# veronicaguerrini/BFQzip

Hardware: AMD Instinct MI355X
Metric: Mbases/s end-to-end (eBWT+cluster+LF), reads and results resident in HBM (higher is better)
Workload: dtype u64

## Files before the change

bfqzip_amd/_lib.py:

```python
import ctypes as C
import os
import subprocess

_HERE = os.path.dirname(os.path.abspath(__file__))
LIB_PATH = os.path.join(_HERE, "libbfqhip.so")
_LIB = None

SYMBOLS = [
    "bfq_default_params", "bfq_create", "bfq_create_error", "bfq_destroy", "bfq_set_params",
    "bfq_last_error", "bfq_stream", "bfq_device_count", "bfq_pick_device", "bfq_device_lease", "bfq_device_release",
    "bfq_phase_enable", "bfq_phase", "bfq_phase_report", "bfq_output_prefault", "bfq_fastq_rows_estimate", "bfq_build_ebwt", "bfq_count_reads",
    "bfq_smooth_invert", "bfq_run_reads", "bfq_run_reads_device", "bfq_fetch_ebwt",
    "bfq_fastq_out_bound", "bfq_fastq_build_ebwt", "bfq_fastq_run", "bfq_fastq_run_streams",
    "bfq_smooth_invert_fastq", "bfq_fastq_run_job", "bfq_host_alloc", "bfq_host_free",
    "bfq_text_count_lines", "bfq_text_nth_newline", "bfq_file_put", "bfq_file_map", "bfq_file_unmap", "bfq_fastq_build_ebwt_fd", "bfq_smooth_invert_fastq_fd",
    "bfq_glob_begin", "bfq_glob_local_text", "bfq_glob_pile_counts", "bfq_glob_init_out", "bfq_glob_run_pile", "bfq_glob_finish",
    "bfq_synth_default", "bfq_synth_total", "bfq_synth_host", "bfq_synth_device", "bfq_synth_fastq",
    "bfq_posbin_geometry", "bfq_radix_geometry", "bfq_prof_enable", "bfq_prof_reset", "bfq_prof_count", "bfq_prof_get", "bfq_prof_trace_select", "bfq_prof_trace",
    "bfq_stream_bound", "bfq_stream_raw_len", "bfq_stream_compress", "bfq_stream_decompress",
    "bfq_stream_reserve", "bfq_stream_compress_device", "bfq_stream_ebwt_decode",
    "bfq_names_compress", "bfq_names_compress_device",
    "bfq_quals_compress", "bfq_quals_compress_device",
    "bfq_fastq_restore_bound", "bfq_fastq_restore", "bfq_fastq_restore_fd",
    "bfq_reorder_key", "bfq_fastq_reorder", "bfq_fastq_reorder_fd",
    "bfq_perm_bound", "bfq_perm_reads", "bfq_perm_encode", "bfq_perm_decode",
    "bfq_fastq_reorder_keep", "bfq_fastq_reorder_keep_fd", "bfq_fastq_unreorder", "bfq_fastq_unreorder_fd",
    "bfq_fastq_restore_ordered", "bfq_fastq_restore_ordered_fd",
    "bfq_fastq_restore_groups", "bfq_stream_members", "bfq_fastq_restore_grouped", "bfq_fastq_restore_grouped_fd",
    "bfq_fastq_compare", "bfq_fastq_compare_fd",
    "bfq_bgzf_probe", "bfq_bgzf_index", "bfq_bgzf_inflate", "bfq_bgzf_inflate_device", "bfq_bgzf_inflate_fd",
    "bfq_bgzf_deflate_bound", "bfq_bgzf_deflate_host", "bfq_bgzf_deflate", "bfq_bgzf_deflate_device", "bfq_bgzf_deflate_fd",
    "bfq_fastq_restore_bgzf_fd",
    "bfq_gzip_probe", "bfq_gzip_measure", "bfq_gzip_inflate", "bfq_gzip_inflate_device", "bfq_gzip_inflate_fd", "bfq_gzip_inflate_host",
# ... 247 lines not shown
        L.bfq_gzip_host_error.restype = C.c_char_p
        L.bfq_gzip_host_error.argtypes = []
        pbo, pbs, a3 = C.POINTER(BamOpts), C.POINTER(BamStats), C.POINTER(u64)
        L.bfq_bam_default_opts.restype = None
        L.bfq_bam_default_opts.argtypes = [pbo]
        L.bfq_bam_probe.argtypes = [vp, u64]
        L.bfq_bam_measure.argtypes = [vp, vp, u64, pbo, a3, a3, pbs]
        L.bfq_bam_to_fastq.argtypes = [vp, vp, u64, pbo, C.POINTER(vp), a3, a3, a3, pbs]
        L.bfq_bam_to_fastq_device.argtypes = [vp, vp, u64, pbo, C.POINTER(vp), a3, a3, a3, pbs]
        L.bfq_bam_to_fastq_fd.argtypes = [vp, C.c_int, u64, pbo, C.POINTER(C.c_int), a3, a3, pbs]
        L.bfq_bam_to_fastq_host.argtypes = [vp, u64, pbo, C.POINTER(vp), a3, a3, a3, pbs]
        L.bfq_bam_host_error.restype = C.c_char_p
        L.bfq_bam_host_error.argtypes = []
        L.bfq_fastq_restore_bgzf_fd.argtypes = [vp, C.c_int, u64, C.c_int, u64, C.c_int, u64, C.c_int, u64, C.c_int, C.c_int, pu64, pu64, pu64]
        L.bfq_posbin_geometry.argtypes = [u64, C.POINTER(u64), C.POINTER(C.c_int)]
        L.bfq_radix_geometry.argtypes = [u64, C.POINTER(u64), C.POINTER(u64)]
        L.bfq_prof_enable.argtypes = [vp, C.c_int]
        L.bfq_prof_reset.argtypes = [vp]
        L.bfq_prof_count.argtypes = [vp]
        L.bfq_prof_trace_select.argtypes = [vp, C.c_int]
        L.bfq_prof_trace.restype = C.c_int64
        L.bfq_prof_trace.argtypes = [vp, vp, u64]
        L.bfq_prof_get.argtypes = [vp, C.c_int, C.c_char_p, C.c_int, C.POINTER(C.c_double),
                                   C.POINTER(u64), C.POINTER(C.c_double)]
        _LIB = L
    return _LIB
```

bfqzip_amd/csrc/bfq_api.hip:

```cpp
#include <math.h>
#include <time.h>
#include <stdlib.h>
#include <stdio.h>
#include <string.h>
#include <unistd.h>
#include <errno.h>
#include <algorithm>
#include <new>
#include "bfq_internal.h"
#include "bfq_synth.h"
#include "bfq_device.h"
#include "bfq_rank.h"
#include "bfq_posbin.h"

const char *const BFQ_KERNEL_NAMES[K_NUM] = {
    "k_text_from_reads", "k_pack3", "k_build_keys", "k_radix_hist", "k_scan", "k_radix_scatter", "k_huge_round",
    "k_cluster_big", "k_refine_chunk", "k_refine_big", "k_emit_bwt", "k_lf_count", "k_lf_build", "k_lcp_flags",
    "k_cluster", "k_invert_count", "k_invert", "k_synth", "k_fastq", "k_bfs", "k_codec", "misc",
    "k_restore_index", "k_fq_format_lines", "k_reorder_keys", "k_reorder_gather",
    "k_fq_format_ordered", "k_perm_pack", "k_perm_invert", "k_posbin_l1", "k_posbin_l2", "k_posbin_apply",
    "k_cmp_check", "k_cmp_compare", "k_cmp_emit", "k_bgzf_inflate", "k_bgzf_deflate"};

static thread_local std::string g_createErr;

void bfq_ctx::reserveBegin(size_t bytes)
{
    bytes = (bytes + 0xFFFFF) & ~(size_t)0xFFFFF;
    if (wsThread || bytes <= ws.cap || (wsLimit() && bytes > wsLimit())) return;
    wsPendBytes = bytes; wsPend = nullptr;
    const int dev = device;
    wsThread = new std::thread([this, dev, bytes] {
        struct timespec t0, t1;
        clock_gettime(CLOCK_MONOTONIC, &t0);
        void *p = nullptr;
        if (hipSetDevice(dev) != hipSuccess || hipMalloc(&p, bytes) != hipSuccess) { (void)hipGetLastError(); p = nullptr; }
        clock_gettime(CLOCK_MONOTONIC, &t1);
// ... 229 lines not shown
extern "C" int64_t bfq_prof_trace(bfq_ctx *c, float *ms, uint64_t cap)
{
    if (!c) return BFQ_E_ARG;
    const size_t k = std::min<size_t>(cap, c->profTrace.size());
    if (ms && k) memcpy(ms, c->profTrace.data(), k * sizeof(float));
    return (int64_t)c->profTrace.size();
}
extern "C" int bfq_prof_count(bfq_ctx *c) { (void)c; return K_NUM; }
extern "C" int bfq_posbin_geometry(uint64_t n_rows, uint64_t *window, int *bin_shift)
{
    const int s = bfq_posbin_shift(n_rows);
    if (window) *window = BFQ_PB_W;
    if (bin_shift) *bin_shift = s;
    return s >= 0 ? BFQ_OK : BFQ_E_ARG;
}
extern "C" int bfq_radix_geometry(uint64_t n_rows, uint64_t *tile_rows, uint64_t *block_rows)
{
    if (tile_rows) *tile_rows = BFQ_RS_TILE;
    if (block_rows) *block_rows = bfq_radix_block_elems(n_rows);
    return BFQ_OK;
}
extern "C" int bfq_prof_get(bfq_ctx *c, int idx, char *name, int cap, double *ms, uint64_t *launches, double *bytes)
{
    if (!c || idx < 0 || idx >= K_NUM) return BFQ_E_ARG;
    if (name && cap > 0) { strncpy(name, BFQ_KERNEL_NAMES[idx], cap - 1); name[cap - 1] = 0; }
    if (ms) *ms = c->profMs[idx];
    if (launches) *launches = c->profLaunches[idx];
    if (bytes) *bytes = c->profBytes[idx];
    return BFQ_OK;
}

static void check_counters(bfq_ctx *c)
{
    const DevCounters &h = c->h_cnt;
    if (h.errSymbol) throw BfqError{BFQ_E_SYMBOL, "symbol outside {A,C,G,T,N,terminator}"};
    if (h.errTooLong) throw BfqError{BFQ_E_TOO_LONG, "read longer than BFQ_MAX_READ_LEN"};
    if (h.errInvert) throw BfqError{BFQ_E_NOT_EBWT, "LF walk did not close: not an eBWT of a read collection"};
    if (h.mismatch) throw BfqError{BFQ_E_NOT_EBWT, "eBWT is not in #_i<#_j<A<C<G<N<T suffix order"};
    if (h.errFreq3) throw BfqError{BFQ_E_FREQ3, "three frequent symbols in a cluster (bfq_int.cpp:505 assert); raise -f"};
}
static void finish_call(bfq_ctx *c, bfq_stats *st = nullptr)
{
    c->fetchCounters();
    c->profCollect();
    check_counters(c);
    if (!st) return;
    const u64 *s = c->h_cnt.stats;
    st->num_clust = s[0]; st->num_clust_discarded = s[1]; st->num_clust_amb_discarded = s[2];
    st->num_clust_mod = s[3]; st->num_clust_alleq = s[4]; st->bases_inside = s[5];
    st->qs_smoothed = s[6]; st->modified = s[7];
    st->n_rows = c->n; st->n_reads = c->N;
    st->n_segments = c->h_cnt.nSegs; st->n_big_segments = c->h_cnt.bigTotal + c->h_cnt.bigCount;
}

static size_t ws_need(u64 n, u64 N, u64 extra)
{
    const u64 nb = ceil_div(n + 1, bfq_radix_block_elems(n)) + 8;
    size_t need = 0;
    need += 4 * (n + 256) + 24 * (n / 256 + 2) + 4096;
    need += 8 * bfq_t3_alloc(n / 21 + 3);
// ... 210 lines not shown
    if (!n) return;
    u8 *dna = c->alloc<u8>(n + 64), *qs = c->alloc<u8>(n + 64);
    if (N) KLAUNCH(c, K_MISC, 4.0 * (double)(n - N), k_lines_init, bfq_grid(N, 16), 256, d_bases, d_quals, d_roff, N, c->P.B, dna, qs);
    u8 *in = c->alloc<u8>(n + 64);
    bfq_lcp_flags(c, c->d_lcp, n, c->P.K, in);
    ClusterPos pm{c->call.d_w12, c->call.d_text3, dna, qs, c->P.B};
    RankIndex none{nullptr, n};
    bfq_clusters(c, none, c->d_bwt, c->d_qual, in, n, &pm);
    if (N) KLAUNCH(c, K_MISC, 4.0 * (double)(n - N), k_lines_strip, bfq_grid(N, 16), 256, (const u8 *)dna, (const u8 *)qs, d_roff, N, d_out_bases, d_out_quals);
}

static size_t posbins_room_needed(u64 n)
{
    const size_t pb = bfq_posbins_need(n);
    if (pb == ~(size_t)0) return pb;
    return pb + 3 * (n + 64 + 256) + 24 * (n / 256 + 8) + (1u << 20);
}
static void steps34_posbins(bfq_ctx *c, const u64 *d_roff, u8 *d_out_bases, u8 *d_out_quals)
{
    const u64 n = c->n, N = c->N;
    if (!n) return;
    u8 *editQual = c->alloc<u8>(n + 64), *repl = c->alloc<u8>(n + 64);
    HIP_CHECK(hipMemcpyAsync(editQual, c->d_qual, n, hipMemcpyDeviceToDevice, c->stream));
    HIP_CHECK(hipMemsetAsync(repl, 0, n + 64, c->stream));
    {
        const size_t mk = c->mark();
        u8 *in = c->alloc<u8>(n + 64);
        bfq_lcp_flags(c, c->d_lcp, n, c->P.K, in);
        ClusterPos pm{c->call.d_w12, c->call.d_text3, nullptr, nullptr, c->P.B, editQual, repl};
        RankIndex none{nullptr, n};
        bfq_clusters(c, none, c->d_bwt, c->d_qual, in, n, &pm);
        c->release(mk);
    }
    bfq_posbins(c, const_cast<u64 *>(c->call.d_w12), repl, editQual, n, d_roff, N, c->P.B, d_out_bases, d_out_quals);
}

static void steps_capped(bfq_ctx *c, const u8 *d_bases, const u8 *d_quals, const u64 *d_roff, u64 N, u64 total, u8 *dna, u8 *qs)
{
    const u64 n = total + N;
    if (n >= (1ull << BFQ_POS_BITS)) throw BfqError{BFQ_E_ARG, "collection too large (2^37 rows)"};
    c->n = n; c->N = N;
    c->d_bwt = c->d_qual = nullptr; c->d_lcp = nullptr; c->d_gcnt = nullptr;
    if (!n) return;
    if (c->P.K < 1) throw BfqError{BFQ_E_NOMEM, "the capped mode needs -k >= 1 (with -k 0 every row is in one cluster): raise the workspace cap"};
// ... 1014 lines not shown
```

bfqzip_amd/csrc/bfq_host.cpp:

```cpp
#include <errno.h>
#include <fcntl.h>
#include <stdio.h>
#include <stdlib.h>
#include <string.h>
#include <sched.h>
#include <sys/file.h>
#include <sys/mman.h>
#include <sys/stat.h>
#include <time.h>
#include <unistd.h>
#include <algorithm>
#include <atomic>
#include <condition_variable>
#include <mutex>
#include <string>
#include <thread>
#include <vector>
#include "bfq_internal_host.h"
#include "bfq_reorder.h"
#include "bfq_perm.h"
#include "bfq_bgzf.h"

static double now_s()
{
// ... 13 lines not shown
            char *end = nullptr;
            double x = strtod(v, &end);
            if (end && (*end == 'G' || *end == 'g')) x *= 1073741824.0;
            else if (end && (*end == 'M' || *end == 'm')) x *= 1048576.0;
            else if (end && (*end == 'K' || *end == 'k')) x *= 1024.0;
            return (unsigned long long)x;
        };
        e.trace = getenv("BFQ_TRACE") != nullptr;
        e.piles = getenv("BFQ_PILES") ? (atoi(getenv("BFQ_PILES")) == 2 ? 2 : atoi(getenv("BFQ_PILES")) ? 1 : -1) : 0;
        e.pilesSplit = getenv("BFQ_PILES_SPLIT") != nullptr;
        e.noOverlap = getenv("BFQ_NO_OVERLAP") != nullptr;
        e.noLengthGuess = getenv("BFQ_NO_LENGTH_GUESS") != nullptr;
        e.posMode = geti("BFQ_POSMODE", 0) != 0;
        e.posBins = geti("BFQ_POSBINS", 1) != 0;
        e.fuseKeys = geti("BFQ_FUSEKEYS", 1) != 0;
        e.ioThreads = geti("BFQ_IO_THREADS", 0);
        e.prefaultThreads = geti("BFQ_PREFAULT_THREADS", -1);
        e.hugeCap = getu("BFQ_HUGE_CAP", 0);
        e.wsCap = getu("BFQ_WS_CAP", 0);
        e.device = getenv("BFQ_DEVICE") ? atoi(getenv("BFQ_DEVICE")) : -1;
        e.fakeDevices = geti("BFQ_FAKE_DEVICES", 0);
        e.lease = geti("BFQ_LEASE", 1) != 0;
        if (const char *d = getenv("BFQ_LEASE_DIR")) e.leaseDir = d;
        e.noOutmap = getenv("BFQ_NO_OUTMAP") != nullptr;
        e.compact = geti("BFQ_COMPACT", 0) != 0;
        e.prefaultPause = geti("BFQ_PREFAULT_PAUSE", 0) != 0;
        e.compactWin = getu("BFQ_COMPACT_WIN", 0);
        e.compactRing = getu("BFQ_COMPACT_RING", 0);
        e.bgzfBatch = getu("BFQ_BGZF_BATCH", 0);
        e.dnaStatic = geti("BFQ_DNA_STATIC", 0);
// ... 536 lines not shown
```

bfqzip_amd/csrc/bfq_internal.h:

```cpp
#pragma once
#include <stdlib.h>
#include <errno.h>
#include <unistd.h>
#include <hip/hip_runtime.h>
#include <stdint.h>
#include <functional>
#include <new>
#include <optional>
#include <string>
#include <vector>
#include <thread>
#include "../../include/bfqzip_hip.h"
#include "bfq_common.h"
#include "bfq_internal_host.h"
#include "bfq_arena.h"

#define HIP_CHECK(expr)                                                                        \
    do {                                                                                       \
        hipError_t e__ = (expr);                                                               \
        if (e__ != hipSuccess)                                                                 \
            throw BfqError{BFQ_E_HIP, std::string(#expr) + ": " + hipGetErrorString(e__)};     \
    } while (0)

enum BfqKernel {
    K_TEXT = 0, K_PACK, K_KEYS, K_RADIX_HIST, K_SCAN, K_RADIX_SCATTER, K_HUGE_ROUND, K_CLUSTER_BIG,
    K_REFINE_WAVE, K_REFINE_BIG, K_EMIT, K_RANK_BUILD, K_RANK_FINAL, K_LCP_FLAGS, K_CLUSTER,
    K_INVERT_COUNT, K_INVERT, K_SYNTH, K_FASTQ, K_BFS, K_CODEC, K_MISC, K_RESTORE, K_FQ_FORMAT, K_RO_KEYS, K_RO_GATHER,
    K_FQ_FORMAT_ORD, K_PERM_PACK, K_PERM_INVERT, K_POSBIN_L1, K_POSBIN_L2, K_POSBIN_APPLY,
    K_CMP_CHECK, K_CMP_COMPARE, K_CMP_EMIT, K_BGZF, K_DEFLATE, K_NUM
};
extern const char *const BFQ_KERNEL_NAMES[K_NUM];

struct ProfRec { int id; hipEvent_t a, b; double bytes; };

#define BFQ_IO_MAX_WORKERS 16
#define BFQ_IO_STAGE_BYTES (16u << 20)

struct DevCounters {
    u64 stats[8];
    u64 bigCount;
    u64 errSymbol;
    u64 errInvert;
    u64 errFreq3;
    u64 errTooLong;
    u64 tot[6];
    u64 mismatch;
    u64 nSegs;
    u64 errFastq;
    u64 hugeCount;
    u64 hugeRows;
    u64 bigClusters;
    u64 bigTotal;
    u64 pad[5];
};

struct RankIndex {
    u64 *lfq;
    u64 n;
};

struct CallState {
    bool piles = false;
    bool capped = false;
    u64 cappedPileRows = 0;
    bool keepRecs = false;
    const u64 *d_w12 = nullptr, *d_text3 = nullptr;
    size_t keepMark = 0;
    size_t writeHint = 0;
// ... 259 lines not shown
struct PileText { u8 *T8, *Q8; u64 *text3; };
void bfq_step1_piles(bfq_ctx *c, const u8 *d_bases, const u8 *d_quals, const u64 *d_roff, u64 N, u64 total, int termOut, bfq_stats *st,
                     const PileText *pre = nullptr, u64 capTarget = 0);
size_t bfq_ws_need_piles(u64 n, u64 N, u64 cap, u64 extra, bool lean = false);
struct PileRows { u64 m; u8 *bwt, *qs; u16 *lcp; const u64 *w12; };
u64 bfq_run_one_pile(bfq_ctx *c, const u8 *T8, const u8 *Q8, const u64 *text3, u64 n, u32 s, u32 s2, int termOut, PileRows *out);
void bfq_pile_pair_counts(bfq_ctx *c, const u8 *T8, u64 n, u64 *counts36);
void bfq_pack_text(bfq_ctx *c, const u8 *T8, u64 n, u64 *text3, u64 nwords);

RankIndex bfq_rank_build(bfq_ctx *c, const u8 *bwt, const u8 *qs, u64 n, int term, const u32 *gcnt = nullptr);
u64 *bfq_symbol_scans(bfq_ctx *c, const u8 *bwt, u64 n, int term, const u32 *gcntIn, u32 *gcntOut);
void bfq_rank_blocks(bfq_ctx *c, const u8 *bwt, u64 n, int term, const u64 *scanned, u64 *rank);
void bfq_lcp_flags(bfq_ctx *c, const u16 *lcp, u64 n, int K, u8 *in);
void bfq_lcp_from_bwt(bfq_ctx *c, const u8 *bwt, u64 n, u64 N, int term, u16 *lcp, u32 *gcntOut = nullptr,
                      const u64 *rankGiven = nullptr, u64 ringEntries = 0);
struct ClusterPos { const u64 *w12; const u64 *text3; u8 *outSym, *outQual; int B; u8 *editQual = nullptr, *repl = nullptr; };
struct ClusterRank { const u64 *rankBlk; u64 F[6]; u8 *qual, *repl; };
void bfq_clusters(bfq_ctx *c, const RankIndex &R, const u8 *bwt, const u8 *qual, const u8 *in, u64 n, const ClusterPos *pm = nullptr,
                  const ClusterRank *rm = nullptr);
#define BFQ_COMPACT_LCP_WIN (256ull << 20)
size_t bfq_ws_need_compact(bfq_ctx *c, u64 n, u64 N, u64 extra, bool haveLcp, size_t resident);
void bfq_steps234_compact(bfq_ctx *c, const u8 *bwt, u8 *qual, HostRef lcp, int lcp_bytes, u64 n, u64 N, u64 *d_roff, u32 *lens,
                          u8 **ob, u8 **oq, u64 extra, size_t resident);
void bfq_invert_count(bfq_ctx *c, const RankIndex &R, u64 N, u32 *lens);
void bfq_fixed_offsets(bfq_ctx *c, u64 N, u64 L, u64 *d_roff);
void bfq_invert(bfq_ctx *c, const RankIndex &R, u64 N, const u64 *d_roff, int B, u8 *out_bases, u8 *out_quals, u64 first = 0,
                u64 count = ~0ull, bool lines = false);
bool bfq_is_pinned(const void *p);
size_t bfq_posbins_need(u64 n);
void bfq_posbins(bfq_ctx *c, u64 *w12, const u8 *repl, const u8 *editQual, u64 n, const u64 *d_roff, u64 N, int B, u8 *outSym, u8 *outQual);

// ... 37 lines not shown
```

bfqzip_amd/csrc/bfq_internal_host.h:

```cpp
#pragma once
#include <stdint.h>
#include <atomic>
#include <string>
#include "../../include/bfqzip_hip.h"

struct BfqError {
    int code;
    std::string msg;
};

struct BfqEnv {
    bool trace = false;
    int piles = 0;
    bool pilesSplit = false;
    bool noOverlap = false;
    bool noLengthGuess = false;
    bool posMode = false;
    bool posBins = true;
    bool fuseKeys = true;
    int ioThreads = 0;
    int prefaultThreads = -1;
    unsigned long long hugeCap = 0;
    unsigned long long wsCap = 0;
    int device = -1;
    int fakeDevices = 0;
    bool lease = true;
    std::string leaseDir;
    bool compact = false;
    int dnaStatic = 0;
    int dnacK = 0, dnacH = 0, dnacW = 0, dnacSkip = -1;
    unsigned long long compactRing = 0;
    unsigned long long compactWin = 0;
    bool prefaultPause = false;
// ... 19 lines not shown
```

bfqzip_amd/csrc/k_cluster.hip:

```cpp
#include <stdlib.h>
#include "bfq_internal.h"
#include "bfq_device.h"
#include "bfq_rank.h"
#include "bfq_rankblk.h"

__global__ __launch_bounds__(256) void k_lcp_flags(const u16 *__restrict__ lcp, u64 n, int K, u8 *__restrict__ in)
{
    const u64 ngroups = (n + 7) / 8;
    for (u64 g = (u64)blockIdx.x * blockDim.x + threadIdx.x; g < ngroups; g += (u64)gridDim.x * blockDim.x) {
        u64 r0 = g * 8;
        int l[10];
        if (r0 >= 1 && r0 + 9 <= n) {
            u64 a = *(const u64 *)(lcp + r0 - 1), b = *(const u64 *)(lcp + r0 + 3);
            u32 c = *(const u32 *)(lcp + r0 + 7);
#pragma unroll
            for (int k = 0; k < 4; k++) { l[k] = (int)((a >> (16 * k)) & 0xFFFF); l[4 + k] = (int)((b >> (16 * k)) & 0xFFFF); }
            l[8] = (int)(c & 0xFFFF); l[9] = (int)(c >> 16);
        } else {
#pragma unroll
            for (int k = 0; k < 10; k++) { u64 r = r0 + k; l[k] = (r >= 1 && r - 1 < n) ? (int)lcp[r - 1] : 0; }
        }
        u64 out = 0;
#pragma unroll
        for (int k = 0; k < 8; k++) {
// ... 183 lines not shown
                else if (ch == symbPrec[1]) { set_mod(a, j, Freq[1]); st.modb++; }
            } else if (b == Freq[0] || b == Freq[1]) {
                set_qual(a, j, newqs); st.qs++;
            } else if (newqs < (int)(signed char)a.qual[j]) {
                set_qual(a, j, newqs); st.qs++;
            }
        }
    } else {
        st.amb++;
    }
    return false;
}

#define CL_CHUNK 4096
#define CL_WROWS (CL_CHUNK / 4)
__global__ __launch_bounds__(256) void k_cluster(ClusterArgs a, u64 nchunks)
{
    __shared__ u32 shst[8];
    __shared__ u16 starts[4][CL_WROWS];
    __shared__ u32 wn[4];
    const u32 lane = bfq_lane(), w = threadIdx.x >> 6;
    if (threadIdx.x < 8) shst[threadIdx.x] = 0;
    ClStat st = {0, 0, 0, 0, 0, 0, 0, 0};
    for (u64 ch = blockIdx.x; ch < nchunks; ch += gridDim.x) {
        const u64 r0 = ch * CL_CHUNK + (u64)w * CL_WROWS + (u64)lane * (CL_WROWS / 64);
        u32 bits = 0;
        if (r0 < a.n) {
            uint4 x = *(const uint4 *)(a.in + r0);
            u32 wds[4] = {x.x, x.y, x.z, x.w};
#pragma unroll
            for (int q = 0; q < 4; q++)
#pragma unroll
                for (int b = 0; b < 4; b++) bits |= ((wds[q] >> (8 * b)) & 1u) << (4 * q + b);
            if (r0 + 16 > a.n) bits &= (1u << (u32)(a.n - r0)) - 1u;
        }
        {
            const u32 zb = ~bits & 0xFFFFu;
            const u64 any = __ballot(zb != 0);
// ... 18 lines not shown
            u64 r = ch * CL_CHUNK + starts[ww][idx];
            if (process_cluster_body(a, r - 1, st)) a.bigStart[atomicAdd(&a.cnt->bigClusters, 1ull)] = r;
        }
        __syncthreads();
    }
    if (st.clust) atomicAdd(&shst[0], st.clust);
    if (st.disc) atomicAdd(&shst[1], st.disc);
    if (st.amb) atomicAdd(&shst[2], st.amb);
    if (st.mod) atomicAdd(&shst[3], st.mod);
    if (st.alleq) atomicAdd(&shst[4], st.alleq);
    if (st.bases) atomicAdd(&shst[5], st.bases);
    if (st.qs) atomicAdd(&shst[6], st.qs);
    if (st.modb) atomicAdd(&shst[7], st.modb);
    __syncthreads();
    if (threadIdx.x < 8 && shst[threadIdx.x]) atomicAdd(&a.cnt->stats[threadIdx.x], (u64)shst[threadIdx.x]);
}

struct BigState {
    u64 start, end;
    u64 freq[5];
    u32 low, sum, mx, fr0, fr1;
    int mode, newqs;
    u32 sym0, sym1;
};
#define CB_TILE 65536
#define CB_GRID 2048

#define CB_FOR_ROWS(...)                                                                               \
    for (u64 g0 = (ts & ~15ull) + (u64)threadIdx.x * 16; g0 <= te; g0 += 256 * 16) {                  \
        const uint4 xb4 = *(const uint4 *)(a.bwt + g0), xq4 = *(const uint4 *)(a.qual + g0);          \
// ... 209 lines not shown
    ClusterArgs a;
    a.R = R; a.bwt = bwt; a.qual = qual; a.in = in; a.n = n;
    a.rankBlk = rm ? rm->rankBlk : nullptr; a.editQual = rm ? rm->qual : pm ? pm->editQual : nullptr; a.repl = rm ? rm->repl : pm ? pm->repl : nullptr;
    for (int s = 0; s < 6; s++) a.F[s] = rm ? rm->F[s] : 0;
    a.w12 = pm ? pm->w12 : nullptr; a.text3 = pm ? pm->text3 : nullptr;
    a.outSym = pm ? pm->outSym : nullptr; a.outQual = pm ? pm->outQual : nullptr; a.B = pm ? pm->B : 0;
    a.m = c->P.m; a.v = c->P.v; a.f = c->P.f; a.t = c->P.t; a.term = c->P.term & 0xFF; a.M = c->P.M; a.ext = c->P.ext;
    a.powtab = c->d_powtab; a.qthr = c->d_qthr; a.qthrLo = c->qthrLo; a.qthrN = c->qthrN;
    a.cnt = c->d_cnt;
    size_t mk = c->mark();
    HIP_CHECK(hipMemsetAsync(&c->d_cnt->bigClusters, 0, sizeof(u64), c->stream));
    a.bigStart = c->alloc<u64>(n / CL_BIG + 2);
    a.big = c->alloc<BigState>(n / CL_BIG + 2);
    a.firstOut = c->alloc<u16>(n / CL_WROWS + 8);
    u64 nchunks = ceil_div(n, CL_CHUNK);
    KLAUNCH(c, K_CLUSTER, 4.125 * (double)n, k_cluster, bfq_grid(nchunks, 1), 256, a, nchunks);
    KLAUNCH(c, K_CLUSTER_BIG, 0.0, k_big_extent, 1024, 256, a);
    KLAUNCH(c, K_CLUSTER_BIG, 0.0, k_big_count, CB_GRID, 256, a);
    KLAUNCH(c, K_CLUSTER_BIG, 0.0, k_big_decide, 64, 256, a);
    KLAUNCH(c, K_CLUSTER_BIG, 0.0, k_big_prec, CB_GRID, 256, a);
    KLAUNCH(c, K_CLUSTER_BIG, 0.0, k_big_apply, CB_GRID, 256, a);
    c->release(mk);
}
```

include/bfqzip_hip.h:

```cpp
#ifndef BFQZIP_HIP_H
#define BFQZIP_HIP_H
#include <stdint.h>
#ifdef __cplusplus
extern "C" {
#endif

#define BFQ_OK              0
#define BFQ_E_ARG          -1
#define BFQ_E_HIP          -2
#define BFQ_E_SYMBOL       -3
#define BFQ_E_NOT_EBWT     -4
#define BFQ_E_TOO_LONG     -5
#define BFQ_E_FREQ3        -6
#define BFQ_E_NOMEM        -7
#define BFQ_E_IO           -8

#define BFQ_MAX_READ_LEN 65000

typedef struct bfq_params {
    int32_t K;
    int32_t m;
    int32_t v;
    int32_t f;
    int32_t t;
// ... 253 lines not shown
uint64_t bfq_bgzf_deflate_bound(uint64_t len);
int bfq_bgzf_deflate_host(const uint8_t *h_in, uint64_t len, int level, uint8_t *h_out, uint64_t cap, uint64_t *out_len);
int bfq_bgzf_deflate(bfq_ctx *c, const uint8_t *h_in, uint64_t len, int level, uint8_t *h_out, uint64_t cap, uint64_t *out_len);
int bfq_bgzf_deflate_device(bfq_ctx *c, const uint8_t *d_in, uint64_t len, int level, uint8_t *h_out, uint64_t cap, uint64_t *out_len);
int bfq_bgzf_deflate_fd(bfq_ctx *c, int in_fd, uint64_t len, int level, int out_fd, uint64_t *out_len);
int bfq_fastq_restore_bgzf_fd(bfq_ctx *c, int dna_fd, uint64_t dna_len, int qs_fd, uint64_t qs_len, int hdr_fd, uint64_t hdr_len,
                              int perm_fd, uint64_t permz_len, int level, int out_fd, uint64_t *out_len, uint64_t *raw_len,
                              uint64_t *n_reads);
int bfq_stream_reserve(bfq_ctx *c, uint64_t len);
int bfq_stream_compress_device(bfq_ctx *c, const uint8_t *d_in, uint64_t len, uint8_t *d_out, uint64_t cap, uint64_t *out_len);

int  bfq_prof_enable(bfq_ctx *c, int on);
void bfq_prof_reset(bfq_ctx *c);
int  bfq_prof_count(bfq_ctx *c);
int  bfq_posbin_geometry(uint64_t n_rows, uint64_t *window, int *bin_shift);
int  bfq_radix_geometry(uint64_t n_rows, uint64_t *tile_rows, uint64_t *block_rows);
int  bfq_prof_get(bfq_ctx *c, int idx, char *name, int name_cap, double *total_ms,
                  uint64_t *launches, double *alg_bytes_total);
int     bfq_prof_trace_select(bfq_ctx *c, int idx);
int64_t bfq_prof_trace(bfq_ctx *c, float *ms, uint64_t cap);

uint64_t bfq_workspace_bytes(bfq_ctx *c);
const char *bfq_version(void);

#ifdef __cplusplus
}
#endif
#endif
```

Measured before the change: 11770.

## Add bitmask-based wave-parallel cluster kernel with deferred fallback for hard clusters

Adds k_cluster_rows, which gives each wave a 1024-row window with 16 rows per lane. It builds per-symbol bitmasks, prefix-scans packed popcount counts across the wave to find cluster extents, and decides and smooths most clusters in registers. It writes editQual and repl directly, which removes the separate device copy and memset on this route. Clusters that leave the window or need the preceding symbols are flagged in a defer bitmap and handled by the original k_cluster body in a second pass. This adds an extra kernel launch and a lot of bit-twiddling complexity for M=2/3, and exactness depends on matching the original decision logic.

Measured after the change: 11570. -1.7%, worse.

```diff
diff --git a/bfqzip_amd/_lib.py b/bfqzip_amd/_lib.py
--- a/bfqzip_amd/_lib.py
+++ b/bfqzip_amd/_lib.py
@@ -16,7 +16,7 @@
     "bfq_text_count_lines", "bfq_text_nth_newline", "bfq_file_put", "bfq_file_map", "bfq_file_unmap", "bfq_fastq_build_ebwt_fd", "bfq_smooth_invert_fastq_fd",
     "bfq_glob_begin", "bfq_glob_local_text", "bfq_glob_pile_counts", "bfq_glob_init_out", "bfq_glob_run_pile", "bfq_glob_finish",
     "bfq_synth_default", "bfq_synth_total", "bfq_synth_host", "bfq_synth_device", "bfq_synth_fastq",
-    "bfq_posbin_geometry", "bfq_radix_geometry", "bfq_prof_enable", "bfq_prof_reset", "bfq_prof_count", "bfq_prof_get", "bfq_prof_trace_select", "bfq_prof_trace",
+    "bfq_posbin_geometry", "bfq_cluster_geometry", "bfq_radix_geometry", "bfq_prof_enable", "bfq_prof_reset", "bfq_prof_count", "bfq_prof_get", "bfq_prof_trace_select", "bfq_prof_trace",
     "bfq_stream_bound", "bfq_stream_raw_len", "bfq_stream_compress", "bfq_stream_decompress",
     "bfq_stream_reserve", "bfq_stream_compress_device", "bfq_stream_ebwt_decode",
     "bfq_names_compress", "bfq_names_compress_device",
@@ -294,6 +294,7 @@
         L.bfq_bam_host_error.argtypes = []
         L.bfq_fastq_restore_bgzf_fd.argtypes = [vp, C.c_int, u64, C.c_int, u64, C.c_int, u64, C.c_int, u64, C.c_int, C.c_int, pu64, pu64, pu64]
         L.bfq_posbin_geometry.argtypes = [u64, C.POINTER(u64), C.POINTER(C.c_int)]
+        L.bfq_cluster_geometry.argtypes = [C.POINTER(u64), C.POINTER(u64)]
         L.bfq_radix_geometry.argtypes = [u64, C.POINTER(u64), C.POINTER(u64)]
         L.bfq_prof_enable.argtypes = [vp, C.c_int]
         L.bfq_prof_reset.argtypes = [vp]
diff --git a/bfqzip_amd/csrc/bfq_api.hip b/bfqzip_amd/csrc/bfq_api.hip
--- a/bfqzip_amd/csrc/bfq_api.hip
+++ b/bfqzip_amd/csrc/bfq_api.hip
@@ -12,6 +12,7 @@
 #include "bfq_device.h"
 #include "bfq_rank.h"
 #include "bfq_posbin.h"
+#include "bfq_cluster_rows.h"
 
 const char *const BFQ_KERNEL_NAMES[K_NUM] = {
     "k_text_from_reads", "k_pack3", "k_build_keys", "k_radix_hist", "k_scan", "k_radix_scatter", "k_huge_round",
@@ -19,7 +20,7 @@
     "k_cluster", "k_invert_count", "k_invert", "k_synth", "k_fastq", "k_bfs", "k_codec", "misc",
     "k_restore_index", "k_fq_format_lines", "k_reorder_keys", "k_reorder_gather",
     "k_fq_format_ordered", "k_perm_pack", "k_perm_invert", "k_posbin_l1", "k_posbin_l2", "k_posbin_apply",
-    "k_cmp_check", "k_cmp_compare", "k_cmp_emit", "k_bgzf_inflate", "k_bgzf_deflate"};
+    "k_cmp_check", "k_cmp_compare", "k_cmp_emit", "k_bgzf_inflate", "k_bgzf_deflate", "k_cluster_rows", "edit_fill"};
 
 static thread_local std::string g_createErr;
 
@@ -279,6 +280,12 @@
     if (bin_shift) *bin_shift = s;
     return s >= 0 ? BFQ_OK : BFQ_E_ARG;
 }
+extern "C" int bfq_cluster_geometry(uint64_t *window_rows, uint64_t *lane_rows)
+{
+    if (window_rows) *window_rows = BFQ_CLR_WROWS;
+    if (lane_rows) *lane_rows = BFQ_CLR_LROWS;
+    return BFQ_OK;
+}
 extern "C" int bfq_radix_geometry(uint64_t n_rows, uint64_t *tile_rows, uint64_t *block_rows)
 {
     if (tile_rows) *tile_rows = BFQ_RS_TILE;
@@ -309,6 +316,9 @@
     c->fetchCounters();
     c->profCollect();
     check_counters(c);
+    if (bfq_env().trace && c->h_cnt.deferred)
+        fprintf(stderr, "[bfq] k_cluster_rows deferred %llu clusters: %llu leave their window, %llu need the preceding symbols\n", (unsigned long long)c->h_cnt.deferred,
+                (unsigned long long)(c->h_cnt.deferred - c->h_cnt.deferredPrec), (unsigned long long)c->h_cnt.deferredPrec);
     if (!st) return;
     const u64 *s = c->h_cnt.stats;
     st->num_clust = s[0]; st->num_clust_discarded = s[1]; st->num_clust_amb_discarded = s[2];
@@ -549,20 +559,25 @@
 {
     const size_t pb = bfq_posbins_need(n);
     if (pb == ~(size_t)0) return pb;
-    return pb + 3 * (n + 64 + 256) + 24 * (n / 256 + 8) + (1u << 20);
+    return pb + 3 * (n + 64 + 256) + 24 * (n / 256 + 8) + (n / 8 + 256) + (1u << 20);
 }
 static void steps34_posbins(bfq_ctx *c, const u64 *d_roff, u8 *d_out_bases, u8 *d_out_quals)
 {
     const u64 n = c->n, N = c->N;
     if (!n) return;
     u8 *editQual = c->alloc<u8>(n + 64), *repl = c->alloc<u8>(n + 64);
-    HIP_CHECK(hipMemcpyAsync(editQual, c->d_qual, n, hipMemcpyDeviceToDevice, c->stream));
-    HIP_CHECK(hipMemsetAsync(repl, 0, n + 64, c->stream));
+    const bool rows = c->env.clusterRows && (c->P.M == 2 || c->P.M == 3);
+    if (!rows) {
+        c->profBegin(K_EDIT_FILL, 3.0 * (double)n);
+        HIP_CHECK(hipMemcpyAsync(editQual, c->d_qual, n, hipMemcpyDeviceToDevice, c->stream));
+        HIP_CHECK(hipMemsetAsync(repl, 0, n + 64, c->stream));
+        c->profEnd();
+    }
     {
         const size_t mk = c->mark();
         u8 *in = c->alloc<u8>(n + 64);
         bfq_lcp_flags(c, c->d_lcp, n, c->P.K, in);
-        ClusterPos pm{c->call.d_w12, c->call.d_text3, nullptr, nullptr, c->P.B, editQual, repl};
+        ClusterPos pm{c->call.d_w12, c->call.d_text3, nullptr, nullptr, c->P.B, editQual, repl, rows};
         RankIndex none{nullptr, n};
         bfq_clusters(c, none, c->d_bwt, c->d_qual, in, n, &pm);
         c->release(mk);
diff --git a/bfqzip_amd/csrc/bfq_cluster_rows.h b/bfqzip_amd/csrc/bfq_cluster_rows.h
--- /dev/null
+++ b/bfqzip_amd/csrc/bfq_cluster_rows.h
@@ -0,0 +1,94 @@
+#pragma once
+#include <math.h>
+#include "bfq_common.h"
+
+#define BFQ_CLR_LROWS 16
+#define BFQ_CLR_WROWS (64 * BFQ_CLR_LROWS)
+#define BFQ_CLR_CBITS 12
+
+BFQ_HD int bfq_clr_ord5(u8 c) { return c == 'A' ? 0 : c == 'C' ? 1 : c == 'G' ? 2 : c == 'T' ? 3 : 4; }
+BFQ_HD u8 bfq_clr_dna5(u32 o) { return (u8)((0x4E54474341ull >> (8u * o)) & 0xFFu); }
+
+struct ClrMasks {
+    u32 sym[5];
+    u32 tr;
+};
+
+BFQ_HD u32 bfq_clr_members(u32 ext) { return (ext | (ext >> 1)) & 0xFFFFu; }
+BFQ_HD u32 bfq_clr_starts(u32 ext) { return ~ext & (ext >> 1) & 0xFFFFu; }
+BFQ_HD u32 bfq_clr_ends(u32 ext) { return ext & ~(ext >> 1) & 0xFFFFu; }
+
+BFQ_HD void bfq_clr_row(ClrMasks &L, u32 k, u8 b, u8 q, bool member, u8 term, int t)
+{
+    const u32 on = (member && b != term) ? 1u : 0u;
+    const u32 isA = b == 'A', isC = b == 'C', isG = b == 'G', isT = b == 'T';
+    L.sym[0] |= (on & isA) << k; L.sym[1] |= (on & isC) << k; L.sym[2] |= (on & isG) << k; L.sym[3] |= (on & isT) << k;
+    L.sym[4] |= (on & ~(isA | isC | isG | isT) & 1u) << k;
+    L.tr |= (on & ((int)(signed char)q >= t + 33 ? 1u : 0u)) << k;
+}
+
+BFQ_HD u64 bfq_clr_pack(const u32 sym[5], u32 range)
+{
+    const u32 lo = (u32)__builtin_popcount(sym[0] & range) | ((u32)__builtin_popcount(sym[1] & range) << BFQ_CLR_CBITS);
+    const u32 hi = (u32)__builtin_popcount(sym[3] & range) | ((u32)__builtin_popcount(sym[4] & range) << BFQ_CLR_CBITS);
+    return (u64)lo | ((u64)(u32)__builtin_popcount(sym[2] & range) << (2 * BFQ_CLR_CBITS)) | ((u64)hi << (3 * BFQ_CLR_CBITS));
+}
+BFQ_HD u32 bfq_clr_field(u64 packed, int o) { return (u32)(packed >> (BFQ_CLR_CBITS * o)) & ((1u << BFQ_CLR_CBITS) - 1u); }
+
+#define BFQ_CLR_NEWQS(d) ((int)(signed char)(u8)((d) & 0xFFu))
+#define BFQ_CLR_SYM(d) (((d) >> 8) & 7u)
+#define BFQ_CLR_LOW(d) (((d) >> 11) & 31u)
+#define BFQ_CLR_SMOOTH (1u << 16)
+#define BFQ_CLR_DEFER (1u << 17)
+#define BFQ_CLR_ST_CLUST (1u << 20)
+#define BFQ_CLR_ST_DISC (1u << 21)
+#define BFQ_CLR_ST_MOD (1u << 22)
+#define BFQ_CLR_ST_ALLEQ (1u << 23)
+#define BFQ_CLR_ST_ERR3 (1u << 24)
+
+BFQ_HD bool bfq_clr_deferred(u32 d) { return (d & BFQ_CLR_DEFER) != 0; }
+
+BFQ_HD u32 bfq_clr_decide(u32 size, u64 cnt, u64 trc, int sum, int m, int f, int v, int M, int ext)
+{
+    if ((u64)size < (u64)(long long)m) return 0;
+    u32 fr[5], bn = 0, low = 0, nnn = 0;
+    for (int o = 0; o < 5; o++) {
+        fr[o] = bfq_clr_field(cnt, o);
+        bn += fr[o];
+        nnn += fr[o] != 0;
+        if (bfq_clr_field(trc, o)) low |= 1u << o;
+    }
+    if (!bn) return BFQ_CLR_ST_CLUST;
+    int newqs;
+    if (M == 2) newqs = (int)(signed char)v;
+    else if (sum == 0) newqs = 0;
+    else if (ext) newqs = (int)(signed char)(u8)roundf((float)sum / (float)bn);
+    else if (sum > 0) newqs = (int)(signed char)(int)((u32)sum / bn);
+    else newqs = (int)(signed char)(int)((u64)(long long)sum / (u64)bn);
+    const int fc = f < 0 ? 0 : f > 101 ? 101 : f;
+    u32 fm = 0;
+    for (int o = 0; o < 5; o++)
+        if (fr[o] && 100u * fr[o] >= (u32)fc * bn) fm |= 1u << o;
+    u32 d = BFQ_CLR_ST_CLUST | (low << 11) | ((u32)newqs & 0xFFu);
+    if (nnn == 1) d |= BFQ_CLR_ST_ALLEQ;
+    const u32 nf = (u32)__builtin_popcount(fm);
+    if (nf >= 3) return d | BFQ_CLR_ST_ERR3;
+    if (nf == 0) return d | BFQ_CLR_ST_DISC;
+    const u32 s0 = (u32)__builtin_ctz(fm);
+    if (nf == 1) return s0 == 4 ? d | BFQ_CLR_ST_DISC : d | BFQ_CLR_SMOOTH | (s0 << 8);
+    if ((u64)bn < (u64)(long long)m) return d | BFQ_CLR_ST_DISC;
+    if (fm & 16u) return d | BFQ_CLR_SMOOTH | BFQ_CLR_ST_MOD | (s0 << 8);
+    return BFQ_CLR_DEFER;
+}
+
+BFQ_HD void bfq_clr_edit(const u32 sym[5], u32 range, u32 d, u32 *repl, u32 *force, u32 *cond)
+{
+    const u32 s = BFQ_CLR_SYM(d), low = BFQ_CLR_LOW(d);
+    u32 rp = 0, cd = 0, fo = 0;
+    for (u32 o = 0; o < 5; o++) {
+        if (o == s) fo |= sym[o];
+        else if ((low >> o) & 1u) cd |= sym[o];
+        else rp |= sym[o];
+    }
+    *repl = rp & range; *cond = cd & range; *force = fo & range;
+}
diff --git a/bfqzip_amd/csrc/bfq_host.cpp b/bfqzip_amd/csrc/bfq_host.cpp
--- a/bfqzip_amd/csrc/bfq_host.cpp
+++ b/bfqzip_amd/csrc/bfq_host.cpp
@@ -51,6 +51,7 @@
         e.posMode = geti("BFQ_POSMODE", 0) != 0;
         e.posBins = geti("BFQ_POSBINS", 1) != 0;
         e.fuseKeys = geti("BFQ_FUSEKEYS", 1) != 0;
+        e.clusterRows = geti("BFQ_CLUSTERROWS", 1) != 0;
         e.ioThreads = geti("BFQ_IO_THREADS", 0);
         e.prefaultThreads = geti("BFQ_PREFAULT_THREADS", -1);
         e.hugeCap = getu("BFQ_HUGE_CAP", 0);
diff --git a/bfqzip_amd/csrc/bfq_internal.h b/bfqzip_amd/csrc/bfq_internal.h
--- a/bfqzip_amd/csrc/bfq_internal.h
+++ b/bfqzip_amd/csrc/bfq_internal.h
@@ -27,7 +27,7 @@
     K_REFINE_WAVE, K_REFINE_BIG, K_EMIT, K_RANK_BUILD, K_RANK_FINAL, K_LCP_FLAGS, K_CLUSTER,
     K_INVERT_COUNT, K_INVERT, K_SYNTH, K_FASTQ, K_BFS, K_CODEC, K_MISC, K_RESTORE, K_FQ_FORMAT, K_RO_KEYS, K_RO_GATHER,
     K_FQ_FORMAT_ORD, K_PERM_PACK, K_PERM_INVERT, K_POSBIN_L1, K_POSBIN_L2, K_POSBIN_APPLY,
-    K_CMP_CHECK, K_CMP_COMPARE, K_CMP_EMIT, K_BGZF, K_DEFLATE, K_NUM
+    K_CMP_CHECK, K_CMP_COMPARE, K_CMP_EMIT, K_BGZF, K_DEFLATE, K_CLUSTER_ROWS, K_EDIT_FILL, K_NUM
 };
 extern const char *const BFQ_KERNEL_NAMES[K_NUM];
 
@@ -51,7 +51,9 @@
     u64 hugeRows;
     u64 bigClusters;
     u64 bigTotal;
-    u64 pad[5];
+    u64 deferred;
+    u64 deferredPrec;
+    u64 pad[3];
 };
 
 struct RankIndex {
@@ -341,7 +343,7 @@
 void bfq_lcp_flags(bfq_ctx *c, const u16 *lcp, u64 n, int K, u8 *in);
 void bfq_lcp_from_bwt(bfq_ctx *c, const u8 *bwt, u64 n, u64 N, int term, u16 *lcp, u32 *gcntOut = nullptr,
                       const u64 *rankGiven = nullptr, u64 ringEntries = 0);
-struct ClusterPos { const u64 *w12; const u64 *text3; u8 *outSym, *outQual; int B; u8 *editQual = nullptr, *repl = nullptr; };
+struct ClusterPos { const u64 *w12; const u64 *text3; u8 *outSym, *outQual; int B; u8 *editQual = nullptr, *repl = nullptr; bool rows = false; };
 struct ClusterRank { const u64 *rankBlk; u64 F[6]; u8 *qual, *repl; };
 void bfq_clusters(bfq_ctx *c, const RankIndex &R, const u8 *bwt, const u8 *qual, const u8 *in, u64 n, const ClusterPos *pm = nullptr,
                   const ClusterRank *rm = nullptr);
diff --git a/bfqzip_amd/csrc/bfq_internal_host.h b/bfqzip_amd/csrc/bfq_internal_host.h
--- a/bfqzip_amd/csrc/bfq_internal_host.h
+++ b/bfqzip_amd/csrc/bfq_internal_host.h
@@ -17,6 +17,7 @@
     bool noLengthGuess = false;
     bool posMode = false;
     bool posBins = true;
+    bool clusterRows = true;
     bool fuseKeys = true;
     int ioThreads = 0;
     int prefaultThreads = -1;
diff --git a/bfqzip_amd/csrc/k_cluster.hip b/bfqzip_amd/csrc/k_cluster.hip
--- a/bfqzip_amd/csrc/k_cluster.hip
+++ b/bfqzip_amd/csrc/k_cluster.hip
@@ -3,6 +3,7 @@
 #include "bfq_device.h"
 #include "bfq_rank.h"
 #include "bfq_rankblk.h"
+#include "bfq_cluster_rows.h"
 
 __global__ __launch_bounds__(256) void k_lcp_flags(const u16 *__restrict__ lcp, u64 n, int K, u8 *__restrict__ in)
 {
@@ -221,7 +222,8 @@
 
 #define CL_CHUNK 4096
 #define CL_WROWS (CL_CHUNK / 4)
-__global__ __launch_bounds__(256) void k_cluster(ClusterArgs a, u64 nchunks)
+template <bool DEFER>
+__global__ __launch_bounds__(256) void k_cluster(ClusterArgs a, u64 nchunks, const u64 *__restrict__ defer)
 {
     __shared__ u32 shst[8];
     __shared__ u16 starts[4][CL_WROWS];
@@ -229,6 +231,13 @@
     const u32 lane = bfq_lane(), w = threadIdx.x >> 6;
     if (threadIdx.x < 8) shst[threadIdx.x] = 0;
     ClStat st = {0, 0, 0, 0, 0, 0, 0, 0};
+    if (DEFER)
+        for (u64 g = (u64)blockIdx.x * 256 + threadIdx.x; g < nchunks; g += (u64)gridDim.x * 256)
+            for (u64 wd = defer[g]; wd; wd &= wd - 1) {
+                const u64 r = g * 64 + (u64)__builtin_ctzll(wd);
+                if (process_cluster_body(a, r - 1, st)) a.bigStart[atomicAdd(&a.cnt->bigClusters, 1ull)] = r;
+            }
+    else
     for (u64 ch = blockIdx.x; ch < nchunks; ch += gridDim.x) {
         const u64 r0 = ch * CL_CHUNK + (u64)w * CL_WROWS + (u64)lane * (CL_WROWS / 64);
         u32 bits = 0;
@@ -277,6 +286,195 @@
     if (st.modb) atomicAdd(&shst[7], st.modb);
     __syncthreads();
     if (threadIdx.x < 8 && shst[threadIdx.x]) atomicAdd(&a.cnt->stats[threadIdx.x], (u64)shst[threadIdx.x]);
+}
+
+static_assert(CL_WROWS == BFQ_CLR_WROWS && CL_WROWS / 64 == BFQ_CLR_LROWS, "one window per wave, 16 rows per lane");
+static_assert(CL_BIG >= CL_WROWS, "a cluster inside one window never belongs to the k_big_* kernels");
+
+__device__ __forceinline__ u32 clr_expand4(u32 nib) { return (((nib & 15u) * 0x00204081u) & 0x01010101u) * 0xFFu; }
+__device__ __forceinline__ int clr_qsum(const u32 xq[4], u32 range)
+{
+    int s = 0;
+#pragma unroll
+    for (int k = 0; k < 16; k++) s += ((range >> k) & 1u) ? (int)(signed char)(u8)(xq[k >> 2] >> (8 * (k & 3))) : 0;
+    return s;
+}
+
+template <bool M3>
+__global__ __launch_bounds__(256) void k_cluster_rows(ClusterArgs a, u16 *__restrict__ defer, u64 nwin)
+{
+    __shared__ u32 shst[11];
+    const u32 lane = bfq_lane();
+    if (threadIdx.x < 11) shst[threadIdx.x] = 0;
+    u32 stClust = 0, stDisc = 0, stMod = 0, stAlleq = 0, stBases = 0, stQs = 0, stModb = 0, stErr3 = 0, stDefer = 0, stPrec = 0;
+    const u8 TERM = (u8)a.term;
+    const u64 ltMask = bfq_lanemask_lt();
+    for (u64 win = (u64)blockIdx.x * 4 + (threadIdx.x >> 6); win < nwin; win += (u64)gridDim.x * 4) {
+        const u64 r0 = win * CL_WROWS + (u64)lane * BFQ_CLR_LROWS;
+        u32 bits = 0;
+        u32 xb[4] = {0, 0, 0, 0}, xq[4] = {0, 0, 0, 0};
+        if (r0 < a.n) {
+            const uint4 x = *(const uint4 *)(a.in + r0), b4 = *(const uint4 *)(a.bwt + r0), q4 = *(const uint4 *)(a.qual + r0);
+            const u32 wds[4] = {x.x, x.y, x.z, x.w};
+            xb[0] = b4.x; xb[1] = b4.y; xb[2] = b4.z; xb[3] = b4.w;
+            xq[0] = q4.x; xq[1] = q4.y; xq[2] = q4.z; xq[3] = q4.w;
+#pragma unroll
+            for (int q = 0; q < 4; q++)
+#pragma unroll
+                for (int b = 0; b < 4; b++) bits |= ((wds[q] >> (8 * b)) & 1u) << (4 * q + b);
+            if (r0 + 16 > a.n) bits &= (1u << (u32)(a.n - r0)) - 1u;
+        }
+        {
+            const u32 zb = ~bits & 0xFFFFu;
+            const u64 any = __ballot(zb != 0);
+            const int fl = any ? __builtin_ctzll(any) : -1;
+            const u32 fz = (u32)__builtin_amdgcn_readlane((int)zb, fl < 0 ? 0 : fl);
+            if (lane == 0) a.firstOut[win] = (u16)(fl < 0 ? CL_WROWS : fl * BFQ_CLR_LROWS + __builtin_ctz(fz));
+        }
+        u32 nextb = (u32)__builtin_amdgcn_update_dpp(0, (int)bits, 0x130, 0xF, 0xF, true) & 1u;
+        if (lane == 63) nextb = (r0 + 16 < a.n) ? (u32)a.in[r0 + 16] & 1u : 0u;
+        const u32 ext = bits | (nextb << 16);
+        const u32 mem = bfq_clr_members(ext), sb = bfq_clr_starts(ext);
+        const u32 eb0 = bfq_clr_ends(ext);
+        u32 eb = eb0;
+
+        ClrMasks L = {{0, 0, 0, 0, 0}, 0};
+#pragma unroll
+        for (int k = 0; k < 16; k++)
+            bfq_clr_row(L, (u32)k, (u8)(xb[k >> 2] >> (8 * (k & 3))), (u8)(xq[k >> 2] >> (8 * (k & 3))), (mem >> k) & 1u, TERM, a.t);
+        const u32 trs[5] = {L.sym[0] & L.tr, L.sym[1] & L.tr, L.sym[2] & L.tr, L.sym[3] & L.tr, L.sym[4] & L.tr};
+        const u32 base = L.sym[0] | L.sym[1] | L.sym[2] | L.sym[3] | L.sym[4];
+
+        const u64 ownC = bfq_clr_pack(L.sym, 0xFFFFu), ownT = bfq_clr_pack(trs, 0xFFFFu);
+        const u64 exC = bfq_wave_incscan64(ownC) - ownC, exT = bfq_wave_incscan64(ownT) - ownT;
+        u32 exS = 0;
+        if (M3) { const u32 ownS = (u32)clr_qsum(xq, base); exS = bfq_wave_incscan32(ownS) - ownS; }
+
+        const u32 sLast = sb ? 31u - (u32)__builtin_clz(sb) : 0u;
+        const u32 below = (1u << sLast) - 1u;
+        const u64 pubC = exC + bfq_clr_pack(L.sym, below), pubT = exT + bfq_clr_pack(trs, below);
+        const u64 hasS = __ballot(sb != 0) & ltMask;
+        const int srcS = hasS ? 63 - __builtin_clzll(hasS) : 0;
+        const u64 carC = ((u64)(u32)__builtin_amdgcn_ds_bpermute(srcS << 2, (int)(u32)(pubC >> 32)) << 32) | (u32)__builtin_amdgcn_ds_bpermute(srcS << 2, (int)(u32)pubC);
+        const u64 carT = ((u64)(u32)__builtin_amdgcn_ds_bpermute(srcS << 2, (int)(u32)(pubT >> 32)) << 32) | (u32)__builtin_amdgcn_ds_bpermute(srcS << 2, (int)(u32)pubT);
+        const u32 carRow = (u32)__builtin_amdgcn_ds_bpermute(srcS << 2, (int)(lane * BFQ_CLR_LROWS + sLast));
+        u32 carS = 0;
+        if (M3) carS = (u32)__builtin_amdgcn_ds_bpermute(srcS << 2, (int)(exS + (u32)clr_qsum(xq, base & below)));
+
+        u32 rp = 0, rs0 = 0, rs1 = 0, force = 0, cond = 0, defStart = 0;
+        u32 nq[4];
+        nq[0] = nq[1] = nq[2] = nq[3] = ((u32)a.v & 0xFFu) * 0x01010101u;
+        auto book = [&](u32 d, u64 cnt) {
+            stClust += (d / BFQ_CLR_ST_CLUST) & 1u; stDisc += (d / BFQ_CLR_ST_DISC) & 1u; stMod += (d / BFQ_CLR_ST_MOD) & 1u;
+            stAlleq += (d / BFQ_CLR_ST_ALLEQ) & 1u; stErr3 += (d / BFQ_CLR_ST_ERR3) & 1u;
+            if (d & BFQ_CLR_ST_CLUST)
+                stBases += bfq_clr_field(cnt, 0) + bfq_clr_field(cnt, 1) + bfq_clr_field(cnt, 2) + bfq_clr_field(cnt, 3) + bfq_clr_field(cnt, 4);
+        };
+        auto apply = [&](u32 d, u32 range) {
+            if (!(d & BFQ_CLR_SMOOTH)) return;
+            u32 r, f, c;
+            bfq_clr_edit(L.sym, range, d, &r, &f, &c);
+            const u32 s = BFQ_CLR_SYM(d);
+            rp |= r; force |= f; cond |= c;
+            if (s & 1u) rs0 |= r;
+            if (s & 2u) rs1 |= r;
+            if (M3) {
+                const u32 q4 = (d & 0xFFu) * 0x01010101u;
+#pragma unroll
+                for (int w = 0; w < 4; w++) { const u32 bm = clr_expand4(range >> (4 * w)); nq[w] = (nq[w] & ~bm) | (q4 & bm); }
+            }
+        };
+
+        u32 d1 = 0;
+        if (eb) {
+            const u32 e = (u32)__builtin_ctz(eb), upto = (2u << e) - 1u, sbel = sb & upto;
+            u32 range = upto, size = 0;
+            u64 cnt = 0, trc = 0;
+            int sum = 0;
+            bool known = true;
+            if (sbel) {
+                const u32 s = 31u - (u32)__builtin_clz(sbel);
+                range = upto & ~((1u << s) - 1u);
+                size = e - s + 1;
+                cnt = bfq_clr_pack(L.sym, range); trc = bfq_clr_pack(trs, range);
+                if (M3) sum = clr_qsum(xq, base & range);
+            } else if (hasS) {
+                size = lane * BFQ_CLR_LROWS + e - carRow + 1;
+                cnt = exC + bfq_clr_pack(L.sym, upto) - carC; trc = exT + bfq_clr_pack(trs, upto) - carT;
+                if (M3) sum = (int)(exS + (u32)clr_qsum(xq, base & upto) - carS);
+            } else known = false;
+            d1 = known ? bfq_clr_decide(size, cnt, trc, sum, a.m, a.f, a.v, M3 ? 3 : 2, a.ext) : BFQ_CLR_DEFER;
+            book(d1, cnt);
+            stPrec += known && bfq_clr_deferred(d1);
+            apply(d1, range);
+            if (sbel && bfq_clr_deferred(d1)) defStart |= 1u << (31u - (u32)__builtin_clz(sbel));
+            eb &= eb - 1;
+        }
+        const u64 hasE = __ballot(eb0 != 0) & ~ltMask & ~(1ull << lane);
+        const int srcE = hasE ? __builtin_ctzll(hasE) : 0;
+        u32 dn = (u32)__builtin_amdgcn_ds_bpermute(srcE << 2, (int)d1);
+        if (!hasE) dn = BFQ_CLR_DEFER;
+
+        while (eb) {
+            const u32 e = (u32)__builtin_ctz(eb), upto = (2u << e) - 1u;
+            const u32 s = 31u - (u32)__builtin_clz(sb & upto);
+            const u32 range = upto & ~((1u << s) - 1u);
+            const u64 cnt = bfq_clr_pack(L.sym, range);
+            const u32 d = bfq_clr_decide(e - s + 1, cnt, bfq_clr_pack(trs, range), M3 ? clr_qsum(xq, base & range) : 0, a.m, a.f, a.v, M3 ? 3 : 2, a.ext);
+            book(d, cnt);
+            apply(d, range);
+            if (bfq_clr_deferred(d)) { defStart |= 1u << s; stPrec++; }
+            eb &= eb - 1;
+        }
+        if (nextb) {
+            apply(dn, sb ? 0xFFFFu & ~below : 0xFFFFu);
+            if (sb && bfq_clr_deferred(dn)) defStart |= 1u << sLast;
+        }
+
+        u32 fb = ((defStart << 1) & 0xFFFFu) | ((u32)__builtin_amdgcn_update_dpp(0, (int)(defStart >> 15), 0x138, 0xF, 0xF, true) & 1u);
+        if (lane == 0) { const u32 prev = (r0 >= 1 && r0 < a.n) ? (u32)a.in[r0 - 1] & 1u : 0u; fb |= bits & ~prev & 1u; }
+        defer[win * 64 + lane] = (u16)fb;
+        stDefer += (u32)__popc(fb);
+
+        u32 lt = 0;
+#pragma unroll
+        for (int k = 0; k < 16; k++)
+            lt |= ((int)(signed char)(u8)(nq[k >> 2] >> (8 * (k & 3))) < (int)(signed char)(u8)(xq[k >> 2] >> (8 * (k & 3))) ? 1u : 0u) << k;
+        const u32 setq = force | (cond & lt);
+        stQs += (u32)__popc(setq); stModb += (u32)__popc(rp);
+        u32 oq[4], orp[4];
+#pragma unroll
+        for (int w = 0; w < 4; w++) {
+            const u32 bm = clr_expand4(setq >> (4 * w));
+            oq[w] = (xq[w] & ~bm) | (nq[w] & bm);
+            const u32 mr = clr_expand4(rp >> (4 * w)), m0 = clr_expand4(rs0 >> (4 * w)), m1 = clr_expand4(rs1 >> (4 * w));
+            orp[w] = (mr & 0x41414141u) ^ (m0 & ~m1 & 0x02020202u) ^ (m1 & ~m0 & 0x06060606u) ^ (m0 & m1 & 0x15151515u);
+        }
+        if (r0 + 16 <= a.n) {
+            *(uint4 *)(a.editQual + r0) = make_uint4(oq[0], oq[1], oq[2], oq[3]);
+            *(uint4 *)(a.repl + r0) = make_uint4(orp[0], orp[1], orp[2], orp[3]);
+        } else if (r0 < a.n) {
+            for (u32 k = 0; k < (u32)(a.n - r0); k++) {
+                a.editQual[r0 + k] = (u8)(oq[k >> 2] >> (8 * (k & 3)));
+                a.repl[r0 + k] = (u8)(orp[k >> 2] >> (8 * (k & 3)));
+            }
+        }
+    }
+    if (stClust) atomicAdd(&shst[0], stClust);
+    if (stDisc) atomicAdd(&shst[1], stDisc);
+    if (stMod) atomicAdd(&shst[3], stMod);
+    if (stAlleq) atomicAdd(&shst[4], stAlleq);
+    if (stBases) atomicAdd(&shst[5], stBases);
+    if (stQs) atomicAdd(&shst[6], stQs);
+    if (stModb) atomicAdd(&shst[7], stModb);
+    if (stErr3) atomicAdd(&shst[8], stErr3);
+    if (stDefer) atomicAdd(&shst[9], stDefer);
+    if (stPrec) atomicAdd(&shst[10], stPrec);
+    __syncthreads();
+    if (threadIdx.x < 8 && shst[threadIdx.x]) atomicAdd(&a.cnt->stats[threadIdx.x], (u64)shst[threadIdx.x]);
+    if (threadIdx.x == 8 && shst[8]) atomicAdd(&a.cnt->errFreq3, (u64)shst[8]);
+    if (threadIdx.x == 9 && shst[9]) atomicAdd(&a.cnt->deferred, (u64)shst[9]);
+    if (threadIdx.x == 10 && shst[10]) atomicAdd(&a.cnt->deferredPrec, (u64)shst[10]);
 }
 
 struct BigState {
@@ -516,7 +714,15 @@
     a.big = c->alloc<BigState>(n / CL_BIG + 2);
     a.firstOut = c->alloc<u16>(n / CL_WROWS + 8);
     u64 nchunks = ceil_div(n, CL_CHUNK);
-    KLAUNCH(c, K_CLUSTER, 4.125 * (double)n, k_cluster, bfq_grid(nchunks, 1), 256, a, nchunks);
+    if (pm && pm->rows) {
+        if (pm->outSym || !pm->editQual || !pm->repl || (a.M != 2 && a.M != 3)) throw BfqError{BFQ_E_ARG, "k_cluster_rows: not the position bins' route"};
+        const u64 nwin = ceil_div(n, CL_WROWS);
+        u16 *defer = c->alloc<u16>(nwin * 64 + 64);
+        if (a.M == 3) KLAUNCH(c, K_CLUSTER_ROWS, 5.0 * (double)n, k_cluster_rows<true>, bfq_grid(nwin, 4), 256, a, defer, nwin);
+        else KLAUNCH(c, K_CLUSTER_ROWS, 5.0 * (double)n, k_cluster_rows<false>, bfq_grid(nwin, 4), 256, a, defer, nwin);
+        KLAUNCH(c, K_CLUSTER, 0.125 * (double)n, k_cluster<true>, bfq_grid(nwin * 16, 256), 256, a, nwin * 16, (const u64 *)defer);
+    } else
+        KLAUNCH(c, K_CLUSTER, 4.125 * (double)n, k_cluster<false>, bfq_grid(nchunks, 1), 256, a, nchunks, (const u64 *)nullptr);
     KLAUNCH(c, K_CLUSTER_BIG, 0.0, k_big_extent, 1024, 256, a);
     KLAUNCH(c, K_CLUSTER_BIG, 0.0, k_big_count, CB_GRID, 256, a);
     KLAUNCH(c, K_CLUSTER_BIG, 0.0, k_big_decide, 64, 256, a);
diff --git a/include/bfqzip_hip.h b/include/bfqzip_hip.h
--- a/include/bfqzip_hip.h
+++ b/include/bfqzip_hip.h
@@ -291,6 +291,7 @@
 void bfq_prof_reset(bfq_ctx *c);
 int  bfq_prof_count(bfq_ctx *c);
 int  bfq_posbin_geometry(uint64_t n_rows, uint64_t *window, int *bin_shift);
+int  bfq_cluster_geometry(uint64_t *window_rows, uint64_t *lane_rows);
 int  bfq_radix_geometry(uint64_t n_rows, uint64_t *tile_rows, uint64_t *block_rows);
 int  bfq_prof_get(bfq_ctx *c, int idx, char *name, int name_cap, double *total_ms,
                   uint64_t *launches, double *alg_bytes_total);
```
